# 0xPARC/plonkathon

Hardware: AMD Instinct MI355X
Metric: proofs/sec at group_order=2^11 (PLONK prover hot path: NTT + quotient + KZG MSM) (higher is better)
Workload: dtype u32x8 (254-bit Montgomery integers, BN254 Fr/Fq); 1 GPU; configs[1]: group_order=2^11, powersOfTau28_hez_final_11 SRS slice, synthetic squaring-chain witness, one distinct witness per proof; lockstep_batch=512, streams_per_gpu=20, parallelism=proof-sharded x1, ranks_in_communicator=1, gather_transport=none (single rank), msm_table_bytes=157571612672

## Files before the change

plonkathon_amd/csrc/fpl.h:

```cpp
#pragma once
#include <math.h>
#include "fp.h"

template <class P>
struct FpL {
    int32_t l[9];
};

#ifdef PLONK_EMU
#include <stdio.h>
#include <stdlib.h>
#define FPL_CHECK(cond, what)                                                       \
    do {                                                                            \
        if (!(cond)) {                                                              \
            fprintf(stderr, "fpl.h range check failed: %s (%s:%d)\n", what, __FILE__, __LINE__); \
            abort();                                                                \
        }                                                                           \
    } while (0)
template <class L> inline long double fpl_dbg_value(const L& a) {
    long double v = 0;
    for (int i = 8; i >= 0; i--) v = v * 536870912.0L + (long double)a.l[i];
    return v;
}
template <class L> inline long long fpl_dbg_maxlimb(const L& a) {
// ... 18 lines not shown
    FPL_CHECK(col < 9223372036854775808.0L, "column sum of a product exceeds 64 bits");
    const long double r_over_m = ldexpl(1.0L, 261) / mm;
    if (!(val <= (r_over_m < 128.0L ? r_over_m : 128.0L) * mm * mm))
        fprintf(stderr, "fpl.h: |a| = %.3Lf m, |b| = %.3Lf m, R / m = %.2Lf\n", fabsl(fpl_dbg_value(a)) / mm, fabsl(fpl_dbg_value(b)) / mm, r_over_m);
    FPL_CHECK(val <= (r_over_m < 128.0L ? r_over_m : 128.0L) * mm * mm, "|a||b| exceeds min(128, R / m) m^2");
}
#define FPL_CHECK_I32(expr64, what) FPL_CHECK((expr64) >= -2147483648LL && (expr64) <= 2147483647LL, what)
#else
#define FPL_CHECK(cond, what) ((void)0)
#define FPL_CHECK_I32(expr64, what) ((void)0)
#endif

#if defined(__HIP_DEVICE_COMPILE__)
#define FPL_ANY_SIGN(x) asm("" : "+v"(x))
#define FPL_ANY_SIGN_UNIFORM(x)                           \
    do {                                                  \
        (x) = __builtin_amdgcn_readfirstlane((int)(x));   \
        asm("" : "+s"(x));                                \
    } while (0)
#else
#define FPL_ANY_SIGN(x) ((void)0)
#define FPL_ANY_SIGN_UNIFORM(x) ((void)0)
#endif

template <class P> PLONK_HD FpL<P> fpl_from_fp(const Fp<P>& a) {
    uint32_t u[9];
    fp29_unpack(a.v, u);
    FpL<P> r;
#pragma unroll
    for (int i = 0; i < 9; i++) {
        r.l[i] = (int32_t)u[i];
        FPL_ANY_SIGN(r.l[i]);
    }
    return r;
}

template <class P> PLONK_HD FpL<P> fpl_from_fp_uniform(const Fp<P>& a) {
    uint32_t u[9];
    fp29_unpack(a.v, u);
    FpL<P> r;
#pragma unroll
    for (int i = 0; i < 9; i++) {
        r.l[i] = (int32_t)u[i];
        FPL_ANY_SIGN_UNIFORM(r.l[i]);
    }
    return r;
}

template <class P> PLONK_HD FpL<P> fpl_zero() {
    FpL<P> r;
#pragma unroll
    for (int i = 0; i < 9; i++) r.l[i] = 0;
    return r;
}

template <class P> PLONK_HD FpL<P> fpl_add(const FpL<P>& a, const FpL<P>& b) {
    FpL<P> r;
#pragma unroll
    for (int i = 0; i < 9; i++) {
        FPL_CHECK_I32((long long)a.l[i] + b.l[i], "fpl_add overflows a limb");
        r.l[i] = a.l[i] + b.l[i];
    }
    return r;
}

template <class P> PLONK_HD FpL<P> fpl_sub(const FpL<P>& a, const FpL<P>& b) {
// ... 466 lines not shown
```

plonkathon_amd/csrc/g1.h:

```cpp
#pragma once
#include "fp.h"

struct alignas(16) G1Affine { Fq x, y; };
struct alignas(16) G1Xyzz { Fq x, y, zz, zzz; };

PLONK_HD bool g1_affine_is_identity(const G1Affine& p) { return fp_is_zero(p.x) && fp_is_zero(p.y); }
PLONK_HD bool g1_is_identity(const G1Xyzz& p) { return fp_is_zero(p.zz); }

PLONK_HD G1Xyzz g1_xyzz_identity() {
    G1Xyzz r;
    r.x = fp_zero<FqParams>(); r.y = fp_zero<FqParams>(); r.zz = fp_zero<FqParams>(); r.zzz = fp_zero<FqParams>();
    return r;
}
PLONK_HD G1Affine g1_affine_identity() {
    G1Affine r;
    r.x = fp_zero<FqParams>(); r.y = fp_zero<FqParams>();
    return r;
}
PLONK_HD G1Xyzz g1_xyzz_from_affine(const G1Affine& p) {
    if (g1_affine_is_identity(p)) return g1_xyzz_identity();
    G1Xyzz r;
    r.x = p.x; r.y = p.y; r.zz = fp_one<FqParams>(); r.zzz = fp_one<FqParams>();
    return r;
}
// ... 106 lines not shown
struct G1XyzzL {
    FqL x, y, zz, zzz;
    bool inf;
};

PLONK_HD G1XyzzL g1l_identity() {
    G1XyzzL r;
#pragma unroll
    for (int i = 0; i < 9; i++) r.x.l[i] = r.y.l[i] = r.zz.l[i] = r.zzz.l[i] = 0;
    r.inf = true;
    return r;
}

PLONK_HD G1Xyzz g1l_to_xyzz(const G1XyzzL& p) {
    if (p.inf) return g1_xyzz_identity();
    G1Xyzz r;
    r.x = fpl_to_fp(p.x);
    r.y = fpl_to_fp(p.y);
    r.zz = fpl_to_fp(p.zz);
    r.zzz = fpl_to_fp(p.zzz);
    return r;
}

PLONK_HD G1XyzzL g1l_from_xyzz(const G1Xyzz& p) {
    G1XyzzL r;
    r.inf = g1_is_identity(p);
    r.x = fpl_from_fp(p.x);
    r.y = fpl_from_fp(p.y);
    r.zz = fpl_from_fp(p.zz);
    r.zzz = fpl_from_fp(p.zzz);
    return r;
}

PLONK_HD bool g1l_madd_fast(G1XyzzL& p, const Fq& x2p, const Fq& y2p, bool neg_y = false) {
    if (fp_is_zero(x2p) && fp_is_zero(y2p)) return false;
    const FqL x2 = fpl_from_fp(x2p), y2 = fpl_cneg(fpl_from_fp(y2p), neg_y);
    if (p.inf) {
        p.x = x2;
        p.y = fpl_norm(y2);
        p.zz = fpl_one<FqParams>();
        p.zzz = p.zz;
        p.inf = false;
        return true;
    }
    const FqL u2 = fpl_mul(x2, p.zz);
    const FqL pp_ = fpl_sub(u2, p.x);
    if (fpl_maybe_zero_mod<FqParams, -5, 8>(pp_)) return false;
    const FqL s2 = fpl_mul(y2, p.zzz);
    const FqL rr = fpl_sub(s2, p.y);
    const FqL pp = fpl_sqr(pp_);
    const FqL q = fpl_mul(p.x, pp);
    p.zz = fpl_mul(p.zz, pp);
    const FqL ppp = fpl_mul(pp_, pp);
    p.zzz = fpl_mul(p.zzz, ppp);
    const FqL r2 = fpl_sqr(rr);
    p.x = fpl_norm(fpl_sub(fpl_sub(r2, ppp), fpl_add(q, q)));
    const FqL d = fpl_sub(q, p.x);
    p.y = fpl_mul_add(rr, d, fpl_neg(p.y), ppp);
    return true;
}

template <bool OPPOSITE_OK = false> PLONK_HD bool g1l_add_fast(G1XyzzL& p, const G1XyzzL& q) {
    if (q.inf) return true;
    if (p.inf) {
        p = q;
        return true;
    }
    const FqL u1 = fpl_mul(p.x, q.zz), u2 = fpl_mul(q.x, p.zz);
    const FqL pp_ = fpl_sub(u2, u1);
    if (fpl_is_zero_mod_in<FqParams, -3, 3>(pp_)) {
        if constexpr (OPPOSITE_OK) {
            const FqL t1 = fpl_mul(p.y, q.zzz), t2 = fpl_mul(q.y, p.zzz);
            if (fpl_is_zero_mod_in<FqParams, -3, 3>(fpl_sub(t2, t1))) return false;
            p = g1l_identity();
            return true;
        }
        return false;
    }
    const FqL s1 = fpl_mul(p.y, q.zzz), s2 = fpl_mul(q.y, p.zzz);
    const FqL rr = fpl_sub(s2, s1);
    const FqL pp = fpl_sqr(pp_);
    const FqL qq = fpl_mul(u1, pp);
    const FqL ppp = fpl_mul(pp_, pp);
    p.zz = fpl_mul(fpl_mul(p.zz, q.zz), pp);
    p.zzz = fpl_mul(fpl_mul(p.zzz, q.zzz), ppp);
    const FqL r2 = fpl_sqr(rr);
    p.x = fpl_norm(fpl_sub(fpl_sub(r2, ppp), fpl_add(qq, qq)));
    const FqL d = fpl_sub(qq, p.x);
    p.y = fpl_mul_add(rr, d, fpl_neg(s1), ppp);
    return true;
}

PLONK_HD void g1l_dbl(G1XyzzL& p) {
// ... 100 lines not shown
```

plonkathon_amd/csrc/msm_comb.h:

```cpp
#pragma once
#include <utility>

#include "msm_common.h"

#define MSM_COMB_MAX_TEETH 24
#define MSM_COMB_SEG_BITS 8
#define MSM_COMB_SCALAR_BITS 254
#define MSM_COMB_REDO 0x80000000u
PLONK_HD bool msm_comb_needs_redo(uint32_t v) { return (v & MSM_COMB_REDO) != 0 || v > MSM_DEFER_CAP; }

PLONK_HD unsigned msm_comb_columns(unsigned h) { return (MSM_COMB_SCALAR_BITS + h - 1) / h; }

struct MsmCombShape {
    unsigned h, a;
    unsigned top_bits, top_g;
    unsigned top_b;
    uint32_t top_entries;
};
PLONK_HD constexpr MsmCombShape msm_comb_shape(unsigned h, bool top) {
    MsmCombShape s{h, (MSM_COMB_SCALAR_BITS + h - 1) / h, 0, 0, 0, 0};
    if (!top) return s;
    s.a = MSM_COMB_SCALAR_BITS / h;
    s.top_bits = MSM_COMB_SCALAR_BITS - s.a * h;
    s.top_b = (2u << s.top_bits) - 1;
    s.top_entries = 1;
    while (s.top_bits && (uint64_t)s.top_entries * s.top_b <= ((uint64_t)1 << (h - 1))) {
        s.top_entries *= s.top_b;
        s.top_g++;
    }
    return s;
}
PLONK_HD constexpr bool msm_comb_top_ok(unsigned h) {
    const MsmCombShape s = msm_comb_shape(h, true);
    return h >= 2 && s.a >= 1 && s.top_bits >= 1 && s.top_bits <= 2 && s.top_g >= 1;
}
PLONK_HD size_t msm_comb_top_groups(size_t n, unsigned g) { return g ? (n + g - 1) / g : 0; }
PLONK_HD size_t msm_comb_virtual(size_t n, const MsmCombShape& s) { return s.top_g ? (msm_comb_top_groups(n, s.top_g) + s.a - 1) / s.a : 0; }
PLONK_HD size_t msm_comb_blocks(size_t n, const MsmCombShape& s) { return n + msm_comb_virtual(n, s) * s.a; }
PLONK_HD bool msm_comb_top_reach_ok(size_t n, const MsmCombShape& s) {
    return !s.top_g || ((uint64_t)(msm_comb_virtual(n, s) * (s.a - 1) + s.a) << (s.h - 1)) < ((uint64_t)1 << 31);
}
PLONK_HD size_t msm_comb_block_of(size_t i, size_t n_real, size_t top_delta) { return i + (i >= n_real ? top_delta : 0); }
// ... 97 lines not shown
    for (size_t id = (size_t)blockIdx.x * blockDim.x + threadIdx.x; id < ng * runs; id += (size_t)gridDim.x * blockDim.x) {
        const size_t bi = id / runs, grp = g0 + bi, i0 = grp * g;
        uint32_t t = (uint32_t)(id - bi * runs);
        G1Xyzz* out = tmp + (bi << hb) + (size_t)t * run;
        G1Xyzz acc = g1_xyzz_identity();
#pragma unroll 1
        for (unsigned pos = low; pos < g; pos++) {
            const int code = (int)(t % B) - (int)c;
            t /= B;
            const G1Affine q = msm_comb_top_point(tq, n, i0 + pos, code < 0);
#pragma unroll 1
            for (int k = 0; k < (code < 0 ? -code : code); k++) g1_madd<true>(acc, q);
        }
        const G1Affine q0 = msm_comb_top_point(tq, n, i0, false), m0 = msm_comb_top_point(tq, n, i0, true);
        const G1Affine q1 = msm_comb_top_point(tq, n, low == 2 ? i0 + 1 : n, false), m1 = msm_comb_top_point(tq, n, low == 2 ? i0 + 1 : n, true);
#pragma unroll 1
        for (unsigned k = 0; k < c; k++) {
            g1_madd<true>(acc, m0);
            g1_madd<true>(acc, m1);
        }
#pragma unroll 1
        for (unsigned d1 = 0; d1 < (low == 2 ? B : 1u); d1++) {
            const bool down = (d1 & 1u) != 0;
#pragma unroll 1
            for (unsigned st = 0; st < B; st++) {
                out[d1 * B + (down ? B - 1 - st : st)] = acc;
                if (st + 1 < B) g1_madd<true>(acc, down ? m0 : q0);
            }
            if (d1 + 1 < B) g1_madd<true>(acc, q1);
        }
    }
}

template <unsigned H, bool TOP> __global__ void __launch_bounds__(256) msm_comb_digits_kernel(const Fr* scalars, size_t n, size_t stride, size_t inner,
                                                                                              size_t outer_stride, size_t m0, uint32_t* digits, size_t nd) {
    constexpr MsmCombShape SH = msm_comb_shape(H, TOP);
    constexpr unsigned A = SH.a, L = A * H;
    static_assert(L <= 9 * 32 && H <= MSM_COMB_MAX_TEETH, "the recoded scalar is kept in nine words");
    constexpr unsigned PER = TOP ? (256 / (SH.top_g ? SH.top_g : 1)) * (SH.top_g ? SH.top_g : 1) : 256;
    const size_t m = m0 + blockIdx.y, i = (size_t)blockIdx.x * PER + threadIdx.x;
    const bool live = threadIdx.x < PER && i < n;
    int code = 0;
    if (live) {
        const Fr* sc = msm_scalar_row(scalars, m, stride, inner, outer_stride);
        const Fr s = fp_load(sc + i);
        const bool even = !(s.v[0] & 1u);
        uint32_t sp[8], br = 0;
#pragma unroll
        for (int k = 0; k < 8; k++) {
            const uint32_t d = fp_sbb(FrParams::mod(k), s.v[k], br);
            sp[k] = even ? d : s.v[k];
        }
        uint32_t w[9];
#pragma unroll
        for (int k = 0; k < 8; k++) w[k] = (sp[k] >> 1) | (k < 7 ? sp[k + 1] << 31 : 0u);
        w[8] = 0;
        if constexpr (TOP) {
            constexpr unsigned hi = L >> 5, sh = L & 31;
            uint32_t u = sp[hi] >> sh;
            if constexpr (sh + SH.top_bits > 32 && hi + 1 < 8) u |= sp[hi + 1] << (32 - sh);
            code = (int)(u & ((1u << SH.top_bits) - 1u));
            if (even) code = -code;
#pragma unroll
            for (unsigned k = 0; k < 9; k++) {
                if (k > ((L - 1) >> 5)) w[k] = 0;
                else if (k == ((L - 1) >> 5)) w[k] &= (1u << ((L - 1) & 31)) - 1u;
            }
        }
        w[(L - 1) >> 5] |= 1u << ((L - 1) & 31);
        uint32_t* out = digits + (m * A) * nd + i;
#pragma unroll
        for (unsigned j = 0; j < A; j++) {
            uint32_t idx = 0;
#pragma unroll
            for (unsigned k = 0; k < H; k++) {
                const unsigned p = j + A * k;
                idx |= ((w[p >> 5] >> (p & 31)) & 1u) << k;
            }
            const uint32_t top = idx >> (H - 1), mask = (1u << (H - 1)) - 1u;
            const uint32_t low = top ? (idx & mask) : (~idx & mask);
            const uint32_t neg = (top ? 0u : 1u) ^ (even ? 1u : 0u);
            out[(size_t)j * nd] = low | (neg << 31);
        }
    }
    if constexpr (TOP) {
        constexpr unsigned G = SH.top_g, B = SH.top_b;
        __shared__ int codes[256];
        codes[threadIdx.x] = code;
        __syncthreads();
        const size_t grp = (size_t)blockIdx.x * (PER / G) + threadIdx.x, nv = msm_comb_virtual(n, SH);
        if (threadIdx.x < PER / G && grp < nv * A) {
            uint32_t idx = 0, pw = 1;
#pragma unroll
            for (unsigned pos = 0; pos < G; pos++) {
                idx += (uint32_t)(codes[threadIdx.x * G + pos] + (int)((B - 1) / 2)) * pw;
                pw *= B;
            }
            const size_t v = grp / A, j = grp - v * A;
            digits[(m * A + j) * nd + n + v] = (uint32_t)((v * (A - 1) + j) << (H - 1)) + idx;
        }
    }
}

struct MsmCombPlan {
    uint32_t q, p, n_main, n_left;
};
PLONK_HD MsmCombPlan msm_comb_plan(uint32_t nsub, uint32_t a) {
    MsmCombPlan pl;
    pl.q = MSM_BLOCK / a;
    pl.p = (a * nsub + MSM_BLOCK - 1) / MSM_BLOCK;
    const uint32_t reach = pl.q * pl.p;
    pl.n_main = reach < nsub ? reach : nsub;
    pl.n_left = nsub - pl.n_main;
    return pl;
}
PLONK_HD void msm_comb_left_pieces(const MsmCombPlan& pl, uint32_t j, uint32_t& ulo, uint32_t& x) {
    if (!pl.n_left) {
        ulo = 0;
        x = 0;
        return;
    }
    ulo = (j * pl.n_left) / pl.p;
    x = ((j + 1) * pl.n_left - 1) / pl.p - ulo + 1;
}
PLONK_HD uint32_t msm_comb_slot(const MsmCombPlan& pl, uint32_t a, uint32_t j, uint32_t r, uint32_t ulo) {
    return r < pl.q ? j * pl.q + r : a * pl.q + ulo + j + (r - pl.q);
}

__global__ void __launch_bounds__(MSM_BLOCK, MSM_ACC_WAVES) msm_comb_kernel(const G1Affine* lookup, unsigned hb, unsigned a,
                                                                             const uint32_t* digits, size_t n, unsigned G,
                                                                             G1Xyzz* partial, MsmDeferred* deferred, size_t deferred_stride,
                                                                             uint32_t* n_deferred, unsigned n_real, unsigned top_delta) {
    PLONK_DYN_SMEM(smem);
    G1Xyzz* red = reinterpret_cast<G1Xyzz*>(smem);
    const unsigned m = blockIdx.x / G, g = blockIdx.x % G, tid = threadIdx.x;
    const uint32_t per_g = (uint32_t)((n + G - 1) / G);
    const uint32_t s0 = g * per_g < n ? g * per_g : (uint32_t)n, s1 = s0 + per_g < n ? s0 + per_g : (uint32_t)n, nsub = s1 - s0;
    const MsmCombPlan pl = msm_comb_plan(nsub, a);
    const uint32_t* dg = digits + (size_t)m * a * n + s0;
    const G1Affine* tab = lookup + ((size_t)s0 << hb);
    const uint32_t nr_rel = n_real > s0 ? n_real - s0 : 0u;
    uint32_t j, i, step, count, slot;
    const bool column_lane = tid < a * pl.q;
    if (column_lane) {
        j = tid / pl.q;
        i = tid - j * pl.q;
        step = pl.q;
        count = i < pl.n_main ? (pl.n_main - 1 - i) / pl.q + 1 : 0;
        slot = tid;
    } else {
        const uint32_t u = tid - a * pl.q, items = a * pl.n_left;
        const uint32_t lo = u * pl.p < items ? u * pl.p : items, hi = lo + pl.p < items ? lo + pl.p : items;
        count = hi - lo;
        j = pl.n_left ? lo / pl.n_left : 0;
        i = pl.n_main + (lo - j * pl.n_left);
        step = 1;
        slot = a * pl.q + u + j;
    }
    G1XyzzL run = g1l_identity();
    auto flush = [&]() { red[slot] = g1l_to_piece(run); };
    for (uint32_t k = 0; k < count; k++) {
        const uint32_t d = dg[(size_t)j * n + i];
        const G1Affine* src = tab + (((size_t)(i + (i >= nr_rel ? top_delta : 0u)) << hb) + (d & 0x7fffffffu));
        const Fq x = fp_load(&src->x), y = fp_load(&src->y);
        if (!g1l_madd_fast(run, x, y, (d >> 31) != 0) && !(fp_is_zero(x) && fp_is_zero(y))) {
            const uint32_t sl = atomicAdd(n_deferred + m, 1u);
            if (sl < MSM_DEFER_CAP) deferred[(size_t)m * deferred_stride + sl] = MsmDeferred{(uint32_t)(j * n + s0 + i), d};
        }
        i += step;
        if (i >= nsub && k + 1 < count) {
            flush();
            run = g1l_identity();
            slot++;
            j++;
            i = pl.n_main;
        }
    }
    if (column_lane || count) flush();
    __syncthreads();
    uint32_t cur = pl.q + (pl.n_left ? (pl.n_left + pl.p - 1) / pl.p + 1 : 0);
    while (cur > 1) {
        const uint32_t half = (cur + 1) / 2, cnt = cur - half;
        for (uint32_t w = tid; w < a * cnt; w += MSM_BLOCK) {
            const uint32_t jj = w / cnt, r = w - jj * cnt;
            uint32_t ulo, x;
            msm_comb_left_pieces(pl, jj, ulo, x);
            if (r + half < pl.q + x) {
                const uint32_t sa = msm_comb_slot(pl, a, jj, r, ulo), sb = msm_comb_slot(pl, a, jj, r + half, ulo);
                const G1XyzzL o = g1l_from_piece(&red[sb]);
                if (!o.inf) {
                    G1XyzzL v = g1l_from_piece(&red[sa]);
                    if (!g1l_add_fast(v, o)) atomicOr(n_deferred + m, MSM_COMB_REDO);
                    red[sa] = g1l_to_piece_wide(v);
                }
            }
        }
        __syncthreads();
        cur = half;
    }
    if (tid < a) partial[((size_t)m * G + g) * a + tid] = red[tid * pl.q];
}

__global__ void __launch_bounds__(64) msm_comb_colsum_kernel(const G1Xyzz* partial, unsigned G, unsigned a, G1Xyzz* colsum, uint32_t* n_deferred) {
    const size_t m = blockIdx.x / a, j = blockIdx.x % a;
    const unsigned lane = threadIdx.x;
    G1XyzzL acc = g1l_identity();
    bool ok = true;
    for (unsigned g = lane; g < G; g += 64) ok &= g1l_add_fast(acc, g1l_from_piece(&partial[(m * G + g) * a + j]));
    ok &= g1l_wave_reduce_step<32>(acc, lane);
    ok &= g1l_wave_reduce_step<16>(acc, lane);
    ok &= g1l_wave_reduce_step<8>(acc, lane);
    ok &= g1l_wave_reduce_step<4>(acc, lane);
    ok &= g1l_wave_reduce_step<2>(acc, lane);
    ok &= g1l_wave_reduce_step<1>(acc, lane);
    if (!ok) atomicOr(n_deferred + m, MSM_COMB_REDO);
    if (lane == 0) colsum[m * a + j] = g1l_to_piece_wide(acc);
}

template <unsigned LPM> __global__ void __launch_bounds__(64) msm_comb_finalize_kernel(const G1Xyzz* sums, size_t M, unsigned G, unsigned a,
                                                                                       const G1Affine* lookup, unsigned hb, size_t n,
                                                                                       const MsmDeferred* deferred, size_t deferred_stride,
                                                                                       uint32_t* n_deferred, Fq* out_xy, uint8_t* flags, unsigned n_real,
                                                                                       unsigned top_delta) {
    const size_t gid = (size_t)blockIdx.x * 64 + threadIdx.x, m = gid / LPM;
    const unsigned l = (unsigned)(gid % LPM), lane = threadIdx.x;
    G1XyzzL acc = g1l_identity();
    bool ok = true;
    if (m < M && l < a) {
        const uint32_t nd = msm_comb_needs_redo(n_deferred[m]) ? 0u : n_deferred[m];
        const unsigned jtop = l + ((a - 1 - l) / LPM) * LPM;
#pragma unroll 1
        for (int j = (int)jtop; j >= 0; j -= (int)LPM) {
            if (j != (int)jtop)
#pragma unroll 1
                for (unsigned d = 0; d < LPM; d++) g1l_dbl(acc);
#pragma unroll 1
            for (unsigned g = 0; g < G; g++) ok &= g1l_add_fast<true>(acc, g1l_from_piece(&sums[(m * G + g) * a + j]));
#pragma unroll 1
            for (uint32_t k = 0; k < nd; k++) {
                const MsmDeferred e = deferred[m * deferred_stride + k];
                if (e.bucket / n != (uint32_t)j) continue;
                const size_t i = e.bucket - (size_t)j * n;
                const G1Affine* src = lookup + ((msm_comb_block_of(i, n_real, top_delta) << hb) + (e.entry & 0x7fffffffu));
                const Fq x = fp_load(&src->x), y = fp_load(&src->y);
                if (!(fp_is_zero(x) && fp_is_zero(y))) ok &= g1l_madd_fast(acc, x, y, (e.entry >> 31) != 0);
            }
        }
#pragma unroll 1
        for (unsigned d = 0; d < l; d++) g1l_dbl(acc);
    }
    if constexpr (LPM >= 2) ok &= g1l_wave_reduce_step<1, true>(acc, lane);
    if constexpr (LPM >= 4) ok &= g1l_wave_reduce_step<2, true>(acc, lane);
    if constexpr (LPM >= 8) ok &= g1l_wave_reduce_step<4, true>(acc, lane);
    if constexpr (LPM >= 16) ok &= g1l_wave_reduce_step<8, true>(acc, lane);
    if constexpr (LPM >= 32) ok &= g1l_wave_reduce_step<16, true>(acc, lane);
    if constexpr (LPM >= 64) ok &= g1l_wave_reduce_step<32, true>(acc, lane);
    if (m < M && !ok) atomicOr(n_deferred + m, MSM_COMB_REDO);
    if (m < M && l == 0) msm_store_result(g1l_to_xyzz(acc), m, out_xy, flags);
}

__global__ void __launch_bounds__(256) msm_comb_slow_kernel(const G1Affine* lookup, unsigned hb, unsigned a, const uint32_t* digits, size_t n,
                                                            const uint32_t* n_deferred, Fq* out_xy, uint8_t* flags, unsigned n_real, unsigned top_delta) {
    __shared__ G1Xyzz red[256];
    const unsigned m = blockIdx.x, tid = threadIdx.x;
    if (!msm_comb_needs_redo(n_deferred[m])) return;
    const uint32_t* dg = digits + (size_t)m * a * n;
    G1Xyzz acc = g1_xyzz_identity();
#pragma unroll 1
    for (int j = (int)a - 1; j >= 0; j--) {
        g1_dbl(acc);
#pragma unroll 1
        for (size_t i = tid; i < n; i += 256) {
            const uint32_t d = dg[(size_t)j * n + i];
            const G1Affine* src = lookup + ((msm_comb_block_of(i, n_real, top_delta) << hb) + (d & 0x7fffffffu));
            G1Affine pt;
            pt.x = fp_load(&src->x);
            pt.y = fp_load(&src->y);
            if (d >> 31) pt.y = fp_neg(pt.y);
            g1_madd<true>(acc, pt);
        }
    }
    msm_fold_store(red, acc, tid, 256, m, out_xy, flags);
}

PLONK_DEV bool msm_comb_entry_matches(const G1Affine& P0, const MsmCombScale& k, unsigned a, unsigned h, uint32_t idx, const G1Affine* e) {
    const G1Affine P = g1_to_affine(msm_comb_scaled_base(P0, k));
    const G1Xyzz v = msm_comb_entry_slow(P, a, h, idx);
    const Fq ex = fp_load(&e->x), ey = fp_load(&e->y);
    if (g1_is_identity(v)) return fp_is_zero(ex) && fp_is_zero(ey);
    return fp_eq(fp_mul(ex, v.zz), v.x) && fp_eq(fp_mul(ey, v.zzz), v.y);
}
__global__ void __launch_bounds__(64) msm_comb_verify_kernel(const G1Affine* bases, const G1Affine* lookup, size_t n, unsigned a, unsigned h,
                                                             unsigned samples, MsmCombScale k, unsigned* mismatches) {
    const size_t t = (size_t)blockIdx.x * blockDim.x + threadIdx.x;
    if (t >= n + 2 * (size_t)samples) return;
    const uint32_t mask = (1u << (h - 1)) - 1u;
    size_t i;
    uint32_t idx;
    if (t < n) {
        i = t;
        idx = mask;
    } else {
        const unsigned s = (unsigned)(t - n) >> 1;
        i = n <= samples ? (s < n ? s : n - 1) : (size_t)s * (n - 1) / (samples - 1);
        idx = ((t - n) & 1) ? (0x55555555u & mask) : 0u;
    }
// ... 19 lines not shown
        b.x = fp_load(&bases[i].x);
        b.y = fp_load(&bases[i].y);
        G1Xyzz p = msm_comb_scaled_base(b, k);
#pragma unroll 1
        for (unsigned d = 0; d < L - j; d++) g1_dbl(p);
        g1_add(sum, p);
    }
    const G1Affine* e = lookup + (((n + grp) << (h - 1)) + idx);
    const Fq ex = fp_load(&e->x), ey = fp_load(&e->y);
    const bool ok = g1_is_identity(sum) ? (fp_is_zero(ex) && fp_is_zero(ey)) : (fp_eq(fp_mul(ex, sum.zz), sum.x) && fp_eq(fp_mul(ey, sum.zzz), sum.y));
    if (!ok) atomicAdd(mismatches, 1u);
}

static size_t msm_comb_stage_entries(size_t n, unsigned h) {
    const size_t half = (size_t)1 << (h - 1);
    size_t bases = n / 8 ? n / 8 : 1;
    while (bases > 1 && bases * half > ((size_t)1 << 27)) bases /= 2;
    return bases * half;
}
static size_t msm_comb_bytes(size_t n, unsigned h, bool top) {
    return (msm_comb_blocks(n, msm_comb_shape(h, top)) << (h - 1)) * sizeof(G1Affine) + msm_comb_stage_entries(n, h) * sizeof(G1Xyzz);
}
static double msm_comb_additions(unsigned h, bool top) {
    const MsmCombShape sh = msm_comb_shape(h, top);
    return (double)sh.a + (top ? 1.0 / sh.top_g : 0.0);
}
bool msm_comb_takes_top(unsigned teeth) { return teeth >= 2 && teeth <= MSM_COMB_MAX_TEETH && msm_comb_top_ok(teeth); }
static bool msm_comb_takes_top_for(size_t n, unsigned h) { return msm_comb_top_ok(h) && msm_comb_top_reach_ok(n, msm_comb_shape(h, true)); }
static bool msm_comb_well_formed(const MsmLookupTable* t) {
    if (t->bits < 2 || t->bits > MSM_COMB_MAX_TEETH) return false;
    const bool top = t->top_g != 0;
    if (top && !msm_comb_top_ok(t->bits)) return false;
    const MsmCombShape sh = msm_comb_shape(t->bits, top);
    return t->windows == sh.a && t->top_bits == sh.top_bits && t->top_g == sh.top_g &&
           t->bytes == (msm_comb_blocks(t->n_points, sh) << (t->bits - 1)) * sizeof(G1Affine);
}

static MsmCombScale msm_comb_scale_constant() {
    Fr one_plain = fp_zero<FrParams>();
    one_plain.v[0] = 1;
    const Fr c = fp_from_mont(one_plain);
    MsmCombScale k;
    for (int i = 0; i < 8; i++) k.c[i] = c.v[i];
    return k;
}

static int msm_comb_build(plonk_ctx* ctx, const plonk_srs* srs, unsigned h, bool top, MsmLookupTable* t) {
    if (top && !msm_comb_top_ok(h)) {
        plonk_set_error("a comb of %u teeth takes no top tables (254 mod teeth must be 1 or 2)", h);
        return PLONK_ERR_ARG;
    }
    const MsmCombShape sh = msm_comb_shape(h, top);
    if (!msm_comb_top_reach_ok(srs->n_points, sh)) {
        plonk_set_error("%zu bases are too many for the top tables of a %u-tooth comb (a virtual scalar's block offset must fit 31 bits)", srs->n_points, h);
        return PLONK_ERR_ARG;
    }
    const unsigned a = sh.a, sb = h - 1 < MSM_COMB_SEG_BITS ? h - 1 : MSM_COMB_SEG_BITS;
    const size_t n = srs->n_points, half = (size_t)1 << (h - 1), stage = msm_comb_stage_entries(n, h), chunk_bases = stage / half;
    const size_t blocks = msm_comb_blocks(n, sh);
    void *gx = nullptr, *gb = nullptr, *dx = nullptr, *db = nullptr, *tmp = nullptr, *tab = nullptr, *pb = nullptr;
    auto fail = [&]() {
        for (void* q : {gx, gb, dx, db, tmp, tab, pb})
            if (q) hipFree(q);
        (void)hipGetLastError();
        plonk_set_error("the %u-tooth comb table (%zu MiB) does not fit in device memory", h, msm_comb_bytes(n, h, top) >> 20);
        return PLONK_ERR_NOMEM;
    };
    if (!plonk_dev_malloc(&tab, blocks * half * sizeof(G1Affine))) return fail();
    if (!plonk_dev_malloc(&tmp, stage * sizeof(G1Xyzz))) return fail();
    if (!plonk_dev_malloc(&gx, n * h * sizeof(G1Xyzz))) return fail();
    if (!plonk_dev_malloc(&gb, n * h * sizeof(G1Affine))) return fail();
    if (!plonk_dev_malloc(&dx, n * (sb ? sb : 1) * sizeof(G1Xyzz))) return fail();
    if (!plonk_dev_malloc(&db, n * (sb ? sb : 1) * sizeof(G1Affine))) return fail();
    if (!plonk_dev_malloc(&pb, n * sizeof(G1Affine))) return fail();
    PLONK_LAUNCH(msm_comb_scale_kernel, grid1(n, 64, 2048), dim3(64), 0, ctx->stream, (const G1Affine*)srs->bases, n, msm_comb_scale_constant(), (G1Xyzz*)gx);
    g1_batch_to_affine(ctx, (const G1Xyzz*)gx, (G1Affine*)pb, n);
    msm_window_bases(ctx, (const G1Affine*)pb, n, a, h, (G1Xyzz*)gx);
    g1_batch_to_affine(ctx, (const G1Xyzz*)gx, (G1Affine*)gb, n * h);
    if (sb) {
        PLONK_LAUNCH(msm_comb_delta_kernel, grid1(n * sb), dim3(256), 0, ctx->stream, (const G1Affine*)gb, n * sb, (G1Xyzz*)dx);
        g1_batch_to_affine(ctx, (const G1Xyzz*)dx, (G1Affine*)db, n * sb);
    }
    for (size_t i0 = 0; i0 < n; i0 += chunk_bases) {
        const size_t nb = n - i0 < chunk_bases ? n - i0 : chunk_bases, lanes = nb << (h - 1 - sb);
        PLONK_LAUNCH(msm_comb_fill_kernel, grid1(lanes, 64, 65536), dim3(64), 0, ctx->stream, (const G1Affine*)gb, (const G1Affine*)db, n, i0, nb, h, sb,
                     (G1Xyzz*)tmp);
        g1_batch_to_affine(ctx, (const G1Xyzz*)tmp, (G1Affine*)tab + i0 * half, nb * half);
    }
    if (top) {
        PLONK_LAUNCH(msm_comb_top_base_kernel, grid1(n, 64, 2048), dim3(64), 0, ctx->stream, (const G1Affine*)pb, n, a * h, a, sh.top_g, (G1Xyzz*)gx);
        g1_batch_to_affine(ctx, (const G1Xyzz*)gx, (G1Affine*)gb, n);
        const size_t groups = msm_comb_top_groups(n, sh.top_g), vblocks = blocks - n, run = sh.top_g >= 2 ? (size_t)sh.top_b * sh.top_b : sh.top_b;
        for (size_t g0 = 0; g0 < vblocks; g0 += chunk_bases) {
            const size_t nb = vblocks - g0 < chunk_bases ? vblocks - g0 : chunk_bases;
            const size_t ng = g0 >= groups ? 0 : (groups - g0 < nb ? groups - g0 : nb);
            if (hipMemsetAsync(tmp, 0, nb * half * sizeof(G1Xyzz), ctx->stream) != hipSuccess) return fail();
            if (ng)
                PLONK_LAUNCH(msm_comb_top_fill_kernel, grid1(ng * (sh.top_entries / run), 64, 65536), dim3(64), 0, ctx->stream, (const G1Affine*)gb, n, g0, ng,
                             h - 1, sh.top_g, sh.top_b, sh.top_entries, (G1Xyzz*)tmp);
            g1_batch_to_affine(ctx, (const G1Xyzz*)tmp, (G1Affine*)tab + (n + g0) * half, nb * half);
        }
    }
    if (hipGetLastError() != hipSuccess || hipStreamSynchronize(ctx->stream) != hipSuccess) return fail();
    for (void* q : {gx, gb, dx, db, tmp, pb}) hipFree(q);
    t->kind = MSM_TABLE_COMB;
    t->bits = h;
    t->windows = a;
    t->top_bits = sh.top_bits;
    t->top_g = sh.top_g;
    t->data = (G1Affine*)tab;
    t->bytes = blocks * half * sizeof(G1Affine);
    return PLONK_OK;
}

static void msm_comb_verify(plonk_ctx* ctx, const plonk_srs* srs, const MsmLookupTable* t, unsigned* d_mismatches) {
    const size_t lanes = srs->n_points + 2 * LUT_VERIFY_SAMPLES;
    PLONK_LAUNCH(msm_comb_verify_kernel, dim3((unsigned)((lanes + 63) / 64)), dim3(64), 0, ctx->stream, (const G1Affine*)srs->bases,
                 (const G1Affine*)t->data, srs->n_points, t->windows, t->bits, (unsigned)LUT_VERIFY_SAMPLES, msm_comb_scale_constant(), d_mismatches);
    if (t->top_g) {
        const size_t groups = msm_comb_top_groups(srs->n_points, t->top_g);
        PLONK_LAUNCH(msm_comb_verify_top_kernel, dim3((unsigned)((groups + 63) / 64)), dim3(64), 0, ctx->stream, (const G1Affine*)srs->bases,
                     (const G1Affine*)t->data, srs->n_points, t->windows, t->bits, t->top_g, (2u << t->top_bits) - 1u, msm_comb_scale_constant(),
                     d_mismatches);
    }
}

template <unsigned H, bool TOP> static void msm_comb_launch_digits(plonk_ctx* ctx, const Fr* d_scalars, size_t n, size_t stride, size_t inner,
                                                                   size_t outer_stride, size_t M, uint32_t* digits, size_t nd) {
    if constexpr (!TOP || msm_comb_top_ok(H)) {
        constexpr MsmCombShape SH = msm_comb_shape(H, TOP);
        constexpr unsigned G = TOP ? SH.top_g : 1, PER = (256 / G) * G;
        size_t gx = (n + PER - 1) / PER;
        if (TOP) {
            const size_t gv = ((nd - n) * SH.a + PER / G - 1) / (PER / G);
            gx = gx > gv ? gx : gv;
        }
        void (*kern)(const Fr*, size_t, size_t, size_t, size_t, size_t, uint32_t*, size_t) = msm_comb_digits_kernel<H, TOP>;
        for (size_t m0 = 0; m0 < M; m0 += 32768) {
            const size_t rows = M - m0 < 32768 ? M - m0 : 32768;
            PLONK_LAUNCH(kern, dim3((unsigned)gx, (unsigned)rows), dim3(256), 0, ctx->stream, d_scalars, n, stride, inner,
                         outer_stride, m0, digits, nd);
        }
    }
}
typedef void (*msm_comb_digits_fn)(plonk_ctx*, const Fr*, size_t, size_t, size_t, size_t, size_t, uint32_t*, size_t);
template <bool TOP, unsigned... H> static msm_comb_digits_fn msm_comb_digits_for(unsigned h, std::integer_sequence<unsigned, H...>) {
    msm_comb_digits_fn fn = nullptr;
    ((h == H + 2 && (!TOP || msm_comb_top_ok(H + 2)) ? (void)(fn = &msm_comb_launch_digits<H + 2, TOP>) : (void)0), ...);
    return fn;
}

static int msm_run_comb(plonk_ctx* ctx, const plonk_srs* srs, const Fr* d_scalars, size_t n_real, size_t M, size_t stride, Fq* d_out_xy, uint8_t* d_flags,
                        size_t inner, size_t outer_stride) {
    const G1Affine* table = srs->shared->data;
    const unsigned h = srs->shared->bits, a = srs->shared->windows, hb = h - 1;
    const bool top = srs->shared->top_g != 0;
    const MsmCombShape sh = msm_comb_shape(h, top);
    const size_t nv = msm_comb_virtual(n_real, sh), n = n_real + nv;
    const unsigned top_delta = (unsigned)(srs->n_points - n_real);
    PLONK_REQUIRE((uint64_t)n * a < ((uint64_t)1 << 32), PLONK_ERR_ARG, "MSM size %zu too large for the lookup path", n_real);
    PLONK_REQUIRE(msm_comb_top_reach_ok(n_real, sh), PLONK_ERR_ARG, "MSM size %zu too large for the top tables of %u teeth", n_real, h);
    unsigned G = msm_groups_per_msm(ctx, M, 64, 3072 / (MSM_BLOCK / 64), 0.035, n * a, 2);
    while (G > 1 && (size_t)G > n) G /= 2;
    MsmScratch s;
    const size_t part_off = s.take(M * G * a * sizeof(G1Xyzz)), col_off = s.take(G >= 4 ? M * a * sizeof(G1Xyzz) : 0), cnt_off = s.take(M * 4);
    const size_t dfr_off = s.take(M * MSM_DEFER_CAP * sizeof(MsmDeferred)), dig_off = s.take(M * a * n * 4);
    PLONK_TRY(ctx_scratch(ctx, 1, s.total, (void**)&s.base));
    G1Xyzz *partial = s.at<G1Xyzz>(part_off), *colsum = s.at<G1Xyzz>(col_off);
    uint32_t *n_deferred = s.at<uint32_t>(cnt_off), *digits = s.at<uint32_t>(dig_off);
    MsmDeferred* deferred = s.at<MsmDeferred>(dfr_off);
    const auto teeth = std::make_integer_sequence<unsigned, MSM_COMB_MAX_TEETH - 1>();
    const msm_comb_digits_fn digits_fn = top ? msm_comb_digits_for<true>(h, teeth) : msm_comb_digits_for<false>(h, teeth);
    PLONK_REQUIRE(digits_fn, PLONK_ERR_ARG, "no comb of %u teeth", h);
    PLONK_CHECK_HIP(hipMemsetAsync(n_deferred, 0, M * 4, ctx->stream));
    PLONK_TRY(prof_begin(ctx, "msm_digits", (double)M * (double)n * (32.0 + 4.0 * a)));
    digits_fn(ctx, d_scalars, n_real, stride, inner, outer_stride, M, digits, n);
    PLONK_TRY(prof_end(ctx));
    const size_t lds = (size_t)(MSM_BLOCK + a) * sizeof(G1Xyzz);
    PLONK_TRY(prof_begin(ctx, "msm_comb", (double)M * (96.0 * (double)n_real + 64.0)));
    PLONK_LAUNCH(msm_comb_kernel, dim3((unsigned)(M * G)), dim3(MSM_BLOCK), lds, ctx->stream, table, hb, a, (const uint32_t*)digits, n, G, partial,
                 deferred, (size_t)MSM_DEFER_CAP, n_deferred, (unsigned)n_real, top_delta);
    PLONK_TRY(prof_end(ctx));
    const G1Xyzz* sums = partial;
    unsigned Gf = G;
    if (G >= 4) {
        PLONK_LAUNCH(msm_comb_colsum_kernel, dim3((unsigned)(M * a)), dim3(64), 0, ctx->stream, (const G1Xyzz*)partial, G, a, colsum, n_deferred);
        sums = colsum;
        Gf = 1;
    }
#define PLONK_COMB_FINALIZE(L)                                                                                                                      \
    PLONK_LAUNCH(msm_comb_finalize_kernel<L>, dim3((unsigned)((M * L + 63) / 64)), dim3(64), 0, ctx->stream, sums, M, Gf, a, table, hb, n,            \
                 (const MsmDeferred*)deferred, (size_t)MSM_DEFER_CAP, n_deferred, d_out_xy, d_flags, (unsigned)n_real, top_delta)
    if (M >= 64) PLONK_COMB_FINALIZE(4);
    else PLONK_COMB_FINALIZE(16);
#undef PLONK_COMB_FINALIZE
    PLONK_LAUNCH(msm_comb_slow_kernel, dim3((unsigned)M), dim3(256), 0, ctx->stream, table, hb, a, (const uint32_t*)digits, n, (const uint32_t*)n_deferred,
                 d_out_xy, d_flags, (unsigned)n_real, top_delta);
    PLONK_CHECK_HIP(hipGetLastError());
    return PLONK_OK;
}

static const MsmTableLayout msm_comb_layout = {22,
                                               msm_comb_takes_top_for,
                                               msm_comb_additions,
                                               msm_comb_bytes,
                                               msm_comb_well_formed,
                                               msm_comb_build,
                                               msm_comb_verify,
                                               msm_run_comb};
```

plonkathon_amd/csrc/msm_tables.h:

```cpp
#pragma once
#include <algorithm>
#include <chrono>
#include <mutex>

#include "msm_comb.h"
#include "msm_windows.h"

static const MsmTableLayout& msm_layout(unsigned kind) { return kind == MSM_TABLE_COMB ? msm_comb_layout : msm_windows_layout; }

static std::mutex g_lut_mu;
static std::vector<MsmLookupTable*> g_luts;

static void lut_attach(plonk_srs* srs, MsmLookupTable* t) {
    if (srs->shared == t) return;
    if (srs->shared && --srs->shared->refs == 0) {
        for (size_t k = 0; k < g_luts.size(); k++)
            if (g_luts[k] == srs->shared) g_luts.erase(g_luts.begin() + k);
        hipFree(srs->shared->data);
        delete srs->shared;
    }
    srs->shared = t;
    if (t) t->refs++;
}

static int lut_build(plonk_ctx* ctx, plonk_srs* srs, unsigned kind, unsigned bits, bool top) {
    const auto t0 = std::chrono::steady_clock::now();
    MsmLookupTable* t = new MsmLookupTable();
    const int rc = msm_layout(kind).build(ctx, srs, bits, top, t);
    if (rc != PLONK_OK) {
        delete t;
        return rc;
    }
    t->device = srs->device;
    t->key = srs->content_key;
    t->n_points = srs->n_points;
    t->build_s = std::chrono::duration<double>(std::chrono::steady_clock::now() - t0).count();
    g_luts.push_back(t);
    lut_attach(srs, t);
    return PLONK_OK;
}

static MsmLookupTable* lut_verified(plonk_ctx* ctx, const plonk_srs* srs, MsmLookupTable* t) {
    if (!t || t->n_points != srs->n_points || !msm_layout(t->kind).well_formed(t)) return nullptr;
    void* flag;
    if (ctx_scratch(ctx, 3, 64, &flag) != PLONK_OK) return nullptr;
    unsigned bad = 1;
    if (hipMemsetAsync(flag, 0, 4, ctx->stream) != hipSuccess) return nullptr;
    msm_layout(t->kind).verify(ctx, srs, t, (unsigned*)flag);
    if (hipMemcpyAsync(&bad, flag, 4, hipMemcpyDeviceToHost, ctx->stream) != hipSuccess || hipStreamSynchronize(ctx->stream) != hipSuccess) return nullptr;
    return bad ? nullptr : t;
}
// ... 115 lines not shown
```

plonkathon_amd/csrc/plonk_internal.h:

```cpp
#pragma once
#include <stdarg.h>
#include <stdio.h>

#include <map>
#include <memory>
#include <string>
#include <vector>

#include "../../include/plonk_hip.h"
#include "fp.h"
#include "g1.h"

void plonk_set_error(const char* fmt, ...);

#define PLONK_CHECK_HIP(expr)                                                                     \
    do {                                                                                          \
        hipError_t e_ = (expr);                                                                   \
        if (e_ != hipSuccess) {                                                                   \
            plonk_set_error("%s failed: %s (%s:%d)", #expr, hipGetErrorString(e_), __FILE__, __LINE__); \
            return PLONK_ERR_HIP;                                                                 \
        }                                                                                         \
    } while (0)

template <class T> static inline bool plonk_dev_malloc(T** p, size_t bytes) {
// ... 58 lines not shown
    do {                         \
        int rc_ = (expr);        \
        if (rc_ != PLONK_OK) return rc_; \
    } while (0)

struct WaveTables {
    std::map<unsigned, int32_t*> prog, lo, hi;
    std::map<unsigned, int32_t*> interpass;
    const int32_t* jm = nullptr;
    bool attr_set[4] = {false, false, false, false};
    std::map<unsigned, void*> packed[3];
    std::map<unsigned, std::shared_ptr<void>> plans;
    unsigned plan_epoch = 0;
};

struct NttTables {
    std::map<unsigned, Fr*> small;
    std::map<unsigned, Fr*> lo, hi;
    std::map<unsigned, Fr*> full;
    WaveTables wave;
};

#define MSM_TABLE_COMB 1
#define MSM_TABLE_WINDOWS 2
struct MsmLookupTable {
    int device = 0;
    uint64_t key = 0;
    size_t n_points = 0;
    unsigned kind = 0;
    unsigned bits = 0, windows = 0;
    unsigned top_bits = 0, top_g = 0;
    G1Affine* data = nullptr;
    size_t bytes = 0;
    double build_s = 0;
    int refs = 0;
};

struct plonk_srs {
    int device = 0;
    uint64_t content_key = 0;
    size_t n_points = 0;
    G1Affine* bases = nullptr;
    unsigned window_bits = 0;
    unsigned n_windows = 0;
    G1Affine* table = nullptr;
    bool fixed = false;
    bool lookup_failed = false;
    MsmLookupTable* shared = nullptr;
    std::map<unsigned, plonk_srs*> lagrange;
    plonk_srs* parent = nullptr;
};

#define PLONK_SCRATCH_SLOTS 4
struct plonk_ctx {
    int device = 0;
    hipStream_t stream = nullptr;
    hipStream_t copy_stream = nullptr;
    NttTables tw;
    std::map<std::string, Fr*> power_tables;
    std::vector<void*> owned;
    void* scratch[PLONK_SCRATCH_SLOTS] = {nullptr, nullptr, nullptr, nullptr};
    size_t scratch_bytes[PLONK_SCRATCH_SLOTS] = {0, 0, 0, 0};
    hipEvent_t ev_a = nullptr, ev_b = nullptr;
    Fr host_tmp[16];
    unsigned msm_window_bits = 0, msm_groups = 0;
    int msm_lookup_mode = 0;
// ... 75 lines not shown
```

Baseline: 50120 proofs/s.

## Skip identity bases and zero top digits in comb MSM, narrow table indexing

Precomputes a per-base skip mask when the comb table is built. The digit kernel uses it to emit a sentinel for identity bases and for neutral top-group entries, so the accumulation kernel skips those table loads and zero checks. The change also folds the y-negation into limb unpacking with a branchless sign mask, and adds a diagonal bit-gather path for digit extraction when there are many teeth. It further uses 32-bit table index arithmetic when the table is small enough, and clears the deferred counters inside the digits kernel in place of a separate memset. The costs are an extra byte array per table and a sentinel check in every deferred and fallback path.

```diff
diff --git a/plonkathon_amd/csrc/fpl.h b/plonkathon_amd/csrc/fpl.h
--- a/plonkathon_amd/csrc/fpl.h
+++ b/plonkathon_amd/csrc/fpl.h
@@ -74,6 +74,21 @@
         r.l[i] = (int32_t)u[i];
         FPL_ANY_SIGN(r.l[i]);
     }
+    return r;
+}
+
+template <class P> PLONK_HD FpL<P> fpl_from_fp_signed(const Fp<P>& a, uint32_t s) {
+    uint32_t v[8], u[9];
+#pragma unroll
+    for (int i = 0; i < 8; i++) v[i] = a.v[i] ^ s;
+    fp29_unpack(v, u);
+    FpL<P> r;
+#pragma unroll
+    for (int i = 0; i < 8; i++) r.l[i] = (int32_t)u[i];
+    r.l[0] -= (int32_t)s;
+    r.l[8] = (int32_t)v[7] >> 8;
+#pragma unroll
+    for (int i = 0; i < 9; i++) FPL_ANY_SIGN(r.l[i]);
     return r;
 }
 
diff --git a/plonkathon_amd/csrc/g1.h b/plonkathon_amd/csrc/g1.h
--- a/plonkathon_amd/csrc/g1.h
+++ b/plonkathon_amd/csrc/g1.h
@@ -162,9 +162,7 @@
     return r;
 }
 
-PLONK_HD bool g1l_madd_fast(G1XyzzL& p, const Fq& x2p, const Fq& y2p, bool neg_y = false) {
-    if (fp_is_zero(x2p) && fp_is_zero(y2p)) return false;
-    const FqL x2 = fpl_from_fp(x2p), y2 = fpl_cneg(fpl_from_fp(y2p), neg_y);
+PLONK_HD bool g1l_madd_limbs(G1XyzzL& p, const FqL& x2, const FqL& y2) {
     if (p.inf) {
         p.x = x2;
         p.y = fpl_norm(y2);
@@ -189,6 +187,13 @@
     p.y = fpl_mul_add(rr, d, fpl_neg(p.y), ppp);
     return true;
 }
+PLONK_HD bool g1l_madd_fast(G1XyzzL& p, const Fq& x2p, const Fq& y2p, bool neg_y = false) {
+    if (fp_is_zero(x2p) && fp_is_zero(y2p)) return false;
+    return g1l_madd_limbs(p, fpl_from_fp(x2p), fpl_cneg(fpl_from_fp(y2p), neg_y));
+}
+PLONK_HD bool g1l_madd_signed(G1XyzzL& p, const Fq& x2p, const Fq& y2p, uint32_t sign) {
+    return g1l_madd_limbs(p, fpl_from_fp(x2p), fpl_from_fp_signed(y2p, sign));
+}
 
 template <bool OPPOSITE_OK = false> PLONK_HD bool g1l_add_fast(G1XyzzL& p, const G1XyzzL& q) {
     if (q.inf) return true;
diff --git a/plonkathon_amd/csrc/msm_comb.h b/plonkathon_amd/csrc/msm_comb.h
--- a/plonkathon_amd/csrc/msm_comb.h
+++ b/plonkathon_amd/csrc/msm_comb.h
@@ -8,6 +8,8 @@
 #define MSM_COMB_SCALAR_BITS 254
 #define MSM_COMB_REDO 0x80000000u
 PLONK_HD bool msm_comb_needs_redo(uint32_t v) { return (v & MSM_COMB_REDO) != 0 || v > MSM_DEFER_CAP; }
+
+#define MSM_COMB_SKIP 0xffffffffu
 
 PLONK_HD unsigned msm_comb_columns(unsigned h) { return (MSM_COMB_SCALAR_BITS + h - 1) / h; }
 
@@ -171,16 +173,28 @@
     }
 }
 
+__global__ void msm_comb_base_skip_kernel(const G1Affine* bases, size_t n, uint8_t* skip) {
+    for (size_t i = (size_t)blockIdx.x * blockDim.x + threadIdx.x; i < n; i += (size_t)gridDim.x * blockDim.x) {
+        G1Affine b;
+        b.x = fp_load(&bases[i].x);
+        b.y = fp_load(&bases[i].y);
+        skip[i] = g1_affine_is_identity(b) ? 1 : 0;
+    }
+}
+
 template <unsigned H, bool TOP> __global__ void __launch_bounds__(256) msm_comb_digits_kernel(const Fr* scalars, size_t n, size_t stride, size_t inner,
-                                                                                              size_t outer_stride, size_t m0, uint32_t* digits, size_t nd) {
+                                                                                              size_t outer_stride, size_t m0, uint32_t* digits, size_t nd,
+                                                                                              const uint8_t* base_skip, uint32_t* n_deferred) {
     constexpr MsmCombShape SH = msm_comb_shape(H, TOP);
     constexpr unsigned A = SH.a, L = A * H;
     static_assert(L <= 9 * 32 && H <= MSM_COMB_MAX_TEETH, "the recoded scalar is kept in nine words");
     constexpr unsigned PER = TOP ? (256 / (SH.top_g ? SH.top_g : 1)) * (SH.top_g ? SH.top_g : 1) : 256;
     const size_t m = m0 + blockIdx.y, i = (size_t)blockIdx.x * PER + threadIdx.x;
     const bool live = threadIdx.x < PER && i < n;
+    if (blockIdx.x == 0 && threadIdx.x == 0) n_deferred[m] = 0;
     int code = 0;
     if (live) {
+        const bool skip = base_skip[i] != 0;
         const Fr* sc = msm_scalar_row(scalars, m, stride, inner, outer_stride);
         const Fr s = fp_load(sc + i);
         const bool even = !(s.v[0] & 1u);
@@ -200,6 +214,7 @@
             if constexpr (sh + SH.top_bits > 32 && hi + 1 < 8) u |= sp[hi + 1] << (32 - sh);
             code = (int)(u & ((1u << SH.top_bits) - 1u));
             if (even) code = -code;
+            if (skip) code = 0;
 #pragma unroll
             for (unsigned k = 0; k < 9; k++) {
                 if (k > ((L - 1) >> 5)) w[k] = 0;
@@ -208,18 +223,48 @@
         }
         w[(L - 1) >> 5] |= 1u << ((L - 1) & 31);
         uint32_t* out = digits + (m * A) * nd + i;
-#pragma unroll
-        for (unsigned j = 0; j < A; j++) {
-            uint32_t idx = 0;
-#pragma unroll
-            for (unsigned k = 0; k < H; k++) {
-                const unsigned p = j + A * k;
-                idx |= ((w[p >> 5] >> (p & 31)) & 1u) << k;
-            }
+        const auto emit = [&](unsigned j, uint32_t idx) PLONK_LAMBDA_INLINE {
             const uint32_t top = idx >> (H - 1), mask = (1u << (H - 1)) - 1u;
             const uint32_t low = top ? (idx & mask) : (~idx & mask);
             const uint32_t neg = (top ? 0u : 1u) ^ (even ? 1u : 0u);
             out[(size_t)j * nd] = low | (neg << 31);
+        };
+        if constexpr (H < 6) {
+#pragma unroll
+            for (unsigned j = 0; j < A; j++) {
+                uint32_t idx = 0;
+#pragma unroll
+                for (unsigned k = 0; k < H; k++) {
+                    const unsigned p = j + A * k;
+                    idx |= ((w[p >> 5] >> (p & 31)) & 1u) << k;
+                }
+                emit(j, idx);
+            }
+        } else {
+            constexpr unsigned C = A < 33 - H ? A : 33 - H;
+#pragma unroll
+            for (unsigned c0 = 0; c0 < A; c0 += C) {
+                uint32_t diag[C] = {};
+#pragma unroll
+                for (unsigned k0 = 0; k0 < C && k0 < H; k0++) {
+                    uint32_t v = 0, teeth = 0;
+#pragma unroll
+                    for (unsigned k = k0; k < H; k += C) {
+                        const unsigned s = (A - 1) * k + c0, q = s >> 5, sh = s & 31;
+                        const uint32_t win = sh ? (w[q] >> sh) | (q + 1 < 9 ? w[q + 1] << (32 - sh) : 0u) : w[q];
+                        v |= win & (((1u << C) - 1u) << k);
+                        teeth |= 1u << k;
+                    }
+#pragma unroll
+                    for (unsigned j = 0; j < C; j++) diag[j] |= v & (teeth << j);
+                }
+#pragma unroll
+                for (unsigned j = c0; j < c0 + C && j < A; j++) emit(j, diag[j - c0] >> (j - c0));
+            }
+        }
+        if (skip) {
+#pragma unroll 1
+            for (unsigned j = 0; j < A; j++) out[(size_t)j * nd] = MSM_COMB_SKIP;
         }
     }
     if constexpr (TOP) {
@@ -236,7 +281,7 @@
                 pw *= B;
             }
             const size_t v = grp / A, j = grp - v * A;
-            digits[(m * A + j) * nd + n + v] = (uint32_t)((v * (A - 1) + j) << (H - 1)) + idx;
+            digits[(m * A + j) * nd + n + v] = idx == (SH.top_entries - 1) / 2 ? MSM_COMB_SKIP : (uint32_t)((v * (A - 1) + j) << (H - 1)) + idx;
         }
     }
 }
@@ -266,6 +311,7 @@
     return r < pl.q ? j * pl.q + r : a * pl.q + ulo + j + (r - pl.q);
 }
 
+template <bool NARROW>
 __global__ void __launch_bounds__(MSM_BLOCK, MSM_ACC_WAVES) msm_comb_kernel(const G1Affine* lookup, unsigned hb, unsigned a,
                                                                              const uint32_t* digits, size_t n, unsigned G,
                                                                              G1Xyzz* partial, MsmDeferred* deferred, size_t deferred_stride,
@@ -298,13 +344,22 @@
     }
     G1XyzzL run = g1l_identity();
     auto flush = [&]() { red[slot] = g1l_to_piece(run); };
+    const uint32_t* col = dg + (size_t)j * n;
     for (uint32_t k = 0; k < count; k++) {
-        const uint32_t d = dg[(size_t)j * n + i];
-        const G1Affine* src = tab + (((size_t)(i + (i >= nr_rel ? top_delta : 0u)) << hb) + (d & 0x7fffffffu));
-        const Fq x = fp_load(&src->x), y = fp_load(&src->y);
-        if (!g1l_madd_fast(run, x, y, (d >> 31) != 0) && !(fp_is_zero(x) && fp_is_zero(y))) {
-            const uint32_t sl = atomicAdd(n_deferred + m, 1u);
-            if (sl < MSM_DEFER_CAP) deferred[(size_t)m * deferred_stride + sl] = MsmDeferred{(uint32_t)(j * n + s0 + i), d};
+        const uint32_t d = col[i];
+        if (d != MSM_COMB_SKIP) {
+            const bool is_virtual = i >= nr_rel;
+            const uint32_t blk = i + (is_virtual ? top_delta : 0u), e = d & 0x7fffffffu;
+            const G1Affine* src;
+            if constexpr (NARROW) src = tab + ((blk << hb) + e);
+            else src = tab + (((size_t)blk << hb) + e);
+            const Fq x = fp_load(&src->x), y = fp_load(&src->y);
+            bool add = true;
+            if (is_virtual) add = !(fp_is_zero(x) && fp_is_zero(y));
+            if (add && !g1l_madd_signed(run, x, y, (uint32_t)((int32_t)d >> 31))) {
+                const uint32_t sl = atomicAdd(n_deferred + m, 1u);
+                if (sl < MSM_DEFER_CAP) deferred[(size_t)m * deferred_stride + sl] = MsmDeferred{(uint32_t)(j * n + s0 + i), d};
+            }
         }
         i += step;
         if (i >= nsub && k + 1 < count) {
@@ -312,6 +367,7 @@
             run = g1l_identity();
             slot++;
             j++;
+            col += n;
             i = pl.n_main;
         }
     }
@@ -378,7 +434,7 @@
 #pragma unroll 1
             for (uint32_t k = 0; k < nd; k++) {
                 const MsmDeferred e = deferred[m * deferred_stride + k];
-                if (e.bucket / n != (uint32_t)j) continue;
+                if (e.bucket / n != (uint32_t)j || e.entry == MSM_COMB_SKIP) continue;
                 const size_t i = e.bucket - (size_t)j * n;
                 const G1Affine* src = lookup + ((msm_comb_block_of(i, n_real, top_delta) << hb) + (e.entry & 0x7fffffffu));
                 const Fq x = fp_load(&src->x), y = fp_load(&src->y);
@@ -411,6 +467,7 @@
 #pragma unroll 1
         for (size_t i = tid; i < n; i += 256) {
             const uint32_t d = dg[(size_t)j * n + i];
+            if (d == MSM_COMB_SKIP) continue;
             const G1Affine* src = lookup + ((msm_comb_block_of(i, n_real, top_delta) << hb) + (d & 0x7fffffffu));
             G1Affine pt;
             pt.x = fp_load(&src->x);
@@ -496,7 +553,7 @@
     const bool top = t->top_g != 0;
     if (top && !msm_comb_top_ok(t->bits)) return false;
     const MsmCombShape sh = msm_comb_shape(t->bits, top);
-    return t->windows == sh.a && t->top_bits == sh.top_bits && t->top_g == sh.top_g &&
+    return t->base_skip && t->windows == sh.a && t->top_bits == sh.top_bits && t->top_g == sh.top_g &&
            t->bytes == (msm_comb_blocks(t->n_points, sh) << (t->bits - 1)) * sizeof(G1Affine);
 }
 
@@ -522,9 +579,9 @@
     const unsigned a = sh.a, sb = h - 1 < MSM_COMB_SEG_BITS ? h - 1 : MSM_COMB_SEG_BITS;
     const size_t n = srs->n_points, half = (size_t)1 << (h - 1), stage = msm_comb_stage_entries(n, h), chunk_bases = stage / half;
     const size_t blocks = msm_comb_blocks(n, sh);
-    void *gx = nullptr, *gb = nullptr, *dx = nullptr, *db = nullptr, *tmp = nullptr, *tab = nullptr, *pb = nullptr;
+    void *gx = nullptr, *gb = nullptr, *dx = nullptr, *db = nullptr, *tmp = nullptr, *tab = nullptr, *pb = nullptr, *skip = nullptr;
     auto fail = [&]() {
-        for (void* q : {gx, gb, dx, db, tmp, tab, pb})
+        for (void* q : {gx, gb, dx, db, tmp, tab, pb, skip})
             if (q) hipFree(q);
         (void)hipGetLastError();
         plonk_set_error("the %u-tooth comb table (%zu MiB) does not fit in device memory", h, msm_comb_bytes(n, h, top) >> 20);
@@ -537,6 +594,8 @@
     if (!plonk_dev_malloc(&dx, n * (sb ? sb : 1) * sizeof(G1Xyzz))) return fail();
     if (!plonk_dev_malloc(&db, n * (sb ? sb : 1) * sizeof(G1Affine))) return fail();
     if (!plonk_dev_malloc(&pb, n * sizeof(G1Affine))) return fail();
+    if (!plonk_dev_malloc(&skip, n)) return fail();
+    PLONK_LAUNCH(msm_comb_base_skip_kernel, grid1(n), dim3(256), 0, ctx->stream, (const G1Affine*)srs->bases, n, (uint8_t*)skip);
     PLONK_LAUNCH(msm_comb_scale_kernel, grid1(n, 64, 2048), dim3(64), 0, ctx->stream, (const G1Affine*)srs->bases, n, msm_comb_scale_constant(), (G1Xyzz*)gx);
     g1_batch_to_affine(ctx, (const G1Xyzz*)gx, (G1Affine*)pb, n);
     msm_window_bases(ctx, (const G1Affine*)pb, n, a, h, (G1Xyzz*)gx);
@@ -573,6 +632,7 @@
     t->top_bits = sh.top_bits;
     t->top_g = sh.top_g;
     t->data = (G1Affine*)tab;
+    t->base_skip = (uint8_t*)skip;
     t->bytes = blocks * half * sizeof(G1Affine);
     return PLONK_OK;
 }
@@ -590,7 +650,8 @@
 }
 
 template <unsigned H, bool TOP> static void msm_comb_launch_digits(plonk_ctx* ctx, const Fr* d_scalars, size_t n, size_t stride, size_t inner,
-                                                                   size_t outer_stride, size_t M, uint32_t* digits, size_t nd) {
+                                                                   size_t outer_stride, size_t M, uint32_t* digits, size_t nd, const uint8_t* base_skip,
+                                                                   uint32_t* n_deferred) {
     if constexpr (!TOP || msm_comb_top_ok(H)) {
         constexpr MsmCombShape SH = msm_comb_shape(H, TOP);
         constexpr unsigned G = TOP ? SH.top_g : 1, PER = (256 / G) * G;
@@ -599,15 +660,15 @@
             const size_t gv = ((nd - n) * SH.a + PER / G - 1) / (PER / G);
             gx = gx > gv ? gx : gv;
         }
-        void (*kern)(const Fr*, size_t, size_t, size_t, size_t, size_t, uint32_t*, size_t) = msm_comb_digits_kernel<H, TOP>;
+        void (*kern)(const Fr*, size_t, size_t, size_t, size_t, size_t, uint32_t*, size_t, const uint8_t*, uint32_t*) = msm_comb_digits_kernel<H, TOP>;
         for (size_t m0 = 0; m0 < M; m0 += 32768) {
             const size_t rows = M - m0 < 32768 ? M - m0 : 32768;
             PLONK_LAUNCH(kern, dim3((unsigned)gx, (unsigned)rows), dim3(256), 0, ctx->stream, d_scalars, n, stride, inner,
-                         outer_stride, m0, digits, nd);
-        }
-    }
-}
-typedef void (*msm_comb_digits_fn)(plonk_ctx*, const Fr*, size_t, size_t, size_t, size_t, size_t, uint32_t*, size_t);
+                         outer_stride, m0, digits, nd, base_skip, n_deferred);
+        }
+    }
+}
+typedef void (*msm_comb_digits_fn)(plonk_ctx*, const Fr*, size_t, size_t, size_t, size_t, size_t, uint32_t*, size_t, const uint8_t*, uint32_t*);
 template <bool TOP, unsigned... H> static msm_comb_digits_fn msm_comb_digits_for(unsigned h, std::integer_sequence<unsigned, H...>) {
     msm_comb_digits_fn fn = nullptr;
     ((h == H + 2 && (!TOP || msm_comb_top_ok(H + 2)) ? (void)(fn = &msm_comb_launch_digits<H + 2, TOP>) : (void)0), ...);
@@ -636,14 +697,15 @@
     const auto teeth = std::make_integer_sequence<unsigned, MSM_COMB_MAX_TEETH - 1>();
     const msm_comb_digits_fn digits_fn = top ? msm_comb_digits_for<true>(h, teeth) : msm_comb_digits_for<false>(h, teeth);
     PLONK_REQUIRE(digits_fn, PLONK_ERR_ARG, "no comb of %u teeth", h);
-    PLONK_CHECK_HIP(hipMemsetAsync(n_deferred, 0, M * 4, ctx->stream));
     PLONK_TRY(prof_begin(ctx, "msm_digits", (double)M * (double)n * (32.0 + 4.0 * a)));
-    digits_fn(ctx, d_scalars, n_real, stride, inner, outer_stride, M, digits, n);
+    digits_fn(ctx, d_scalars, n_real, stride, inner, outer_stride, M, digits, n, srs->shared->base_skip, n_deferred);
     PLONK_TRY(prof_end(ctx));
     const size_t lds = (size_t)(MSM_BLOCK + a) * sizeof(G1Xyzz);
     PLONK_TRY(prof_begin(ctx, "msm_comb", (double)M * (96.0 * (double)n_real + 64.0)));
-    PLONK_LAUNCH(msm_comb_kernel, dim3((unsigned)(M * G)), dim3(MSM_BLOCK), lds, ctx->stream, table, hb, a, (const uint32_t*)digits, n, G, partial,
-                 deferred, (size_t)MSM_DEFER_CAP, n_deferred, (unsigned)n_real, top_delta);
+    const bool narrow = srs->shared->bytes / sizeof(G1Affine) <= ((uint64_t)1 << 32);
+    const auto comb_kernel = narrow ? msm_comb_kernel<true> : msm_comb_kernel<false>;
+    PLONK_LAUNCH(comb_kernel, dim3((unsigned)(M * G)), dim3(MSM_BLOCK), lds, ctx->stream, table, hb, a,
+                 (const uint32_t*)digits, n, G, partial, deferred, (size_t)MSM_DEFER_CAP, n_deferred, (unsigned)n_real, top_delta);
     PLONK_TRY(prof_end(ctx));
     const G1Xyzz* sums = partial;
     unsigned Gf = G;
diff --git a/plonkathon_amd/csrc/msm_tables.h b/plonkathon_amd/csrc/msm_tables.h
--- a/plonkathon_amd/csrc/msm_tables.h
+++ b/plonkathon_amd/csrc/msm_tables.h
@@ -17,6 +17,7 @@
         for (size_t k = 0; k < g_luts.size(); k++)
             if (g_luts[k] == srs->shared) g_luts.erase(g_luts.begin() + k);
         hipFree(srs->shared->data);
+        hipFree(srs->shared->base_skip);
         delete srs->shared;
     }
     srs->shared = t;
diff --git a/plonkathon_amd/csrc/plonk_internal.h b/plonkathon_amd/csrc/plonk_internal.h
--- a/plonkathon_amd/csrc/plonk_internal.h
+++ b/plonkathon_amd/csrc/plonk_internal.h
@@ -114,6 +114,7 @@
     unsigned top_bits = 0, top_g = 0;
     G1Affine* data = nullptr;
     size_t bytes = 0;
+    uint8_t* base_skip = nullptr;
     double build_s = 0;
     int refs = 0;
 };
```

Result: faster. 50790 proofs/s (median of 6 runs) (+1.3%).
